# marwie/mageslam

Hardware: AMD Instinct MI355X
Metric: frames/sec ORB extract+match @720p; local-BA iters/sec (50 KF, 5k pts) (higher is better)
Workload: dtype u8

## Files before the change

### mageslam_amd/csrc/orb.hip

```cpp
#include <hip/hip_runtime.h>

#include <algorithm>
#include <cmath>
#include <cstring>
#include <type_traits>
#include <vector>

#include "common.hpp"
#include "cv_rng.hpp"
#include "fast_tile_plan.hpp"
#include "lds_sort.hpp"
#include "orb_tables.hpp"

namespace mage {
namespace {

constexpr int TW = 120, TH = 30;
constexpr int GX = (TW + 8) / 4;
constexpr int SR = 8;
constexpr int SROWS = TH + 2;
constexpr int LW = TW + 16;
constexpr int LH = TH + 8;
constexpr int FAST_THREADS = GX * (SROWS / SR);
constexpr int TCAP = (TW / 2) * (TH / 2);
// ... 11 lines not shown
    int dword_ok;
    int qword_ok;
    uint8_t* blur;
    int blur_stride;
    long long blur_pitch;
    int blur_bcols;
    const uint4* blur_ops;
    const int* gate;
    int* gate_next;
    uint32_t* redo;
};

struct Tile {
    int x, y;
};

__device__ __forceinline__ void wave_lds_sync()
{
    __builtin_amdgcn_fence(__ATOMIC_RELEASE, "wavefront");
    __builtin_amdgcn_wave_barrier();
    __builtin_amdgcn_fence(__ATOMIC_ACQUIRE, "wavefront");
}

typedef _Float16 h2 __attribute__((ext_vector_type(2)));
__device__ __forceinline__ h2 as_h2(uint32_t u) { return __builtin_bit_cast(h2, u); }
__device__ __forceinline__ uint32_t as_u32(h2 h) { return __builtin_bit_cast(uint32_t, h); }
__device__ __forceinline__ h2 min3h(h2 a, h2 b, h2 c)
{
    return __builtin_elementwise_minimum(__builtin_elementwise_minimum(a, b), c);
}
__device__ __forceinline__ h2 max3h(h2 a, h2 b, h2 c)
{
    return __builtin_elementwise_maximum(__builtin_elementwise_maximum(a, b), c);
}

__device__ __forceinline__ h2 pair_in(uint32_t d, int k)
{
    return as_h2(__builtin_amdgcn_perm(d, 0x64646464u, (uint32_t)((4 + k) | ((5 + k) << 16))));
}
__device__ __forceinline__ h2 pair_cross(uint32_t lo, uint32_t hi)
{
    return as_h2(__builtin_amdgcn_perm(hi, lo, 0x0C040C03u) | 0x64006400u);
}

__device__ __forceinline__ void window_row(uint32_t d0, uint32_t d1, uint32_t d2, h2 (&q)[9])
{
// ... 73 lines not shown
}

__device__ __forceinline__ int reflect101(int i, int n)
{
    if (n == 1) return 0;
    while ((unsigned)i >= (unsigned)n) i = i < 0 ? -i : 2 * n - 2 - i;
    return i;
}

typedef uint32_t u32x4 __attribute__((ext_vector_type(4)));
__device__ __forceinline__ u32x4 shr_bytes(u32x4 a, int s)
{
    if (s & 8) a = u32x4{a[2], a[3], 0u, 0u};
    if (s & 4) a = u32x4{a[1], a[2], a[3], 0u};
    const uint32_t b = (uint32_t)s & 3u;
    return u32x4{__builtin_amdgcn_alignbyte(a[1], a[0], b), __builtin_amdgcn_alignbyte(a[2], a[1], b),
                 __builtin_amdgcn_alignbyte(a[3], a[2], b), __builtin_amdgcn_alignbyte(0u, a[3], b)};
}
__device__ __forceinline__ u32x4 rev_bytes(u32x4 a)
{
    return u32x4{__builtin_bswap32(a[3]), __builtin_bswap32(a[2]), __builtin_bswap32(a[1]), __builtin_bswap32(a[0])};
}

__device__ __noinline__ void load_tile_border(const uint8_t* __restrict__ src_, int w_, int h_, int stride_,
                                              uint8_t (*img)[LW], int gx0_, int gy0_)
{
    const int w = __builtin_amdgcn_readfirstlane(w_), h = __builtin_amdgcn_readfirstlane(h_);
    const int stride = __builtin_amdgcn_readfirstlane(stride_);
    const int gx0 = __builtin_amdgcn_readfirstlane(gx0_), gy0 = __builtin_amdgcn_readfirstlane(gy0_);
    const unsigned long long sa = (unsigned long long)src_;
    const unsigned long long sb = ((unsigned long long)(uint32_t)__builtin_amdgcn_readfirstlane((int)(sa >> 32)) << 32) |
                                  (uint32_t)__builtin_amdgcn_readfirstlane((int)sa);
    typedef const __attribute__((address_space(1))) uint8_t* gptr;
    typedef uint32_t u32x2 __attribute__((ext_vector_type(2)));
    typedef const __attribute__((address_space(1))) u32x2 __attribute__((aligned(1))) g_u2;
    typedef const __attribute__((address_space(1))) u32x4 __attribute__((aligned(1))) g_u4;
    const gptr src = (gptr)sb;
    static_assert(LW == tileplan::kLW && LH == tileplan::kLH, "the plan's tile window");
    constexpr int RSTEP = FAST_THREADS / 9, NPASS = (LH + RSTEP - 1) / RSTEP;
    const int c = threadIdx.x % 9, r0 = threadIdx.x / 9;
    if (r0 >= RSTEP) return;
    if (gx0 + LW <= w) {
        const bool left = gx0 < 0 && c == 0;
        const gptr gc = src + (left ? 0 : gx0 + (c < 8 ? 16 * c : 120));
        u32x4 v[NPASS];
#pragma unroll
        for (int k = 0; k < NPASS; k++)
            if (r0 + k * RSTEP < LH)
                v[k] = *(g_u4*)(gc + (long long)tileplan::mirror1(gy0 + r0 + k * RSTEP, h) * stride);
#pragma unroll
        for (int k = 0; k < NPASS; k++) {
            const int r = r0 + k * RSTEP;
            if (r >= LH) break;
            u32x4 t = v[k];
            if (left)
                t = u32x4{__builtin_amdgcn_perm(t[2], t[1], 0x01020304u), __builtin_amdgcn_perm(t[1], t[0], 0x01020304u),
                          t[0], t[1]};
            uint2* d = reinterpret_cast<uint2*>(&img[r][16 * c]);
            if (c < 8) {
                d[0] = make_uint2(t[0], t[1]);
                d[1] = make_uint2(t[2], t[3]);
            } else {
                d[0] = make_uint2(t[2], t[3]);
// ... 21 lines not shown
#pragma unroll
        for (int k = 0; k < NPASS; k++) {
            const int r = r0 + k * RSTEP;
            if (r >= LH) break;
            const u32x4 t = v[k];
            u32x4 o;
            if (cp.kind == tileplan::CHUNK_STRADDLE) {
                o = shr_bytes(t, 16 - cp.n) | rev_bytes(shr_bytes(t, cp.n - 1));
            } else if (cp.kind == tileplan::CHUNK_MIRROR) {
                o = half ? u32x4{__builtin_bswap32(t[1]), __builtin_bswap32(t[0]), 0u, 0u} : rev_bytes(t);
            } else if (cp.kind == tileplan::CHUNK_LEFT) {
                o = u32x4{__builtin_amdgcn_perm(t[2], t[1], 0x01020304u), __builtin_amdgcn_perm(t[1], t[0], 0x01020304u),
                          t[0], t[1]};
            } else {
                o = c < 8 ? t : u32x4{t[2], t[3], 0u, 0u};
            }
            uint2* d = reinterpret_cast<uint2*>(&img[r][16 * c]);
            d[0] = make_uint2(o[0], o[1]);
            if (c < 8) d[1] = make_uint2(o[2], o[3]);
        }
    }
}

__device__ __forceinline__ void load_tile(const uint8_t* __restrict__ src, const FastParams& p,
                                          uint8_t (*img)[LW], Tile T)
{
    const int gx0 = T.x * TW - 8, gy0 = T.y * TH - 4;
    if (p.qword_ok && gx0 >= 0 && gx0 + LW <= p.w && gy0 >= 0 && gy0 + LH <= p.h) {
        static_assert(LW == 8 * 16 + 8, "row = 8 x 16 + 8 bytes");
        constexpr int RSTEP = FAST_THREADS / 9, NPASS = (LH + RSTEP - 1) / RSTEP;
        const int c = threadIdx.x % 9, r0 = threadIdx.x / 9;
        if (r0 < RSTEP) {
            const uint8_t* g = src + (long long)(gy0 + r0) * p.stride + gx0 + (c < 8 ? 16 * c : 120);
            const long long gstep = (long long)RSTEP * p.stride;
            typedef uint32_t u32x4 __attribute__((ext_vector_type(4)));
            u32x4 v[NPASS];
#pragma unroll
            for (int k = 0; k < NPASS; k++)
                if (r0 + k * RSTEP < LH) __builtin_memcpy(&v[k], g + k * gstep, 16);
#pragma unroll
            for (int k = 0; k < NPASS; k++) {
                const int r = r0 + k * RSTEP;
                if (r >= LH) break;
                if (c < 8) {
                    uint2* d = reinterpret_cast<uint2*>(&img[r][16 * c]);
                    d[0] = make_uint2(v[k][0], v[k][1]);
                    d[1] = make_uint2(v[k][2], v[k][3]);
                } else {
                    *reinterpret_cast<uint2*>(&img[r][128]) = make_uint2(v[k][2], v[k][3]);
                }
            }
        }
        return;
    }
    if (p.qword_ok && tileplan::border_ok(p.w, p.h, gx0, gy0)) {
        load_tile_border(src, p.w, p.h, p.stride, img, gx0, gy0);
        return;
    }
    constexpr int DW = LW / 4;
    for (int i = threadIdx.x; i < LH * DW; i += FAST_THREADS) {
        const int r = i / DW, c = i - r * DW;
        const int gx = gx0 + 4 * c, gy = reflect101(gy0 + r, p.h);
        const uint8_t* row = src + (long long)gy * p.stride;
        uint32_t v;
        if (p.dword_ok && gx >= 0 && gx + 3 < p.w) {
            v = *reinterpret_cast<const uint32_t*>(row + gx);
        } else {
            v = 0;
#pragma unroll
            for (int q = 0; q < 4; q++) v |= (uint32_t)row[reflect101(gx + q, p.w)] << (8 * q);
        }
        *reinterpret_cast<uint32_t*>(&img[r][4 * c]) = v;
    }
}

__device__ __forceinline__ void score_strip(const uint8_t (*img)[LW], uint32_t (*sc)[GX], const FastParams& p, Tile T)
{
    const int gx = threadIdx.x % GX, chunk = threadIdx.x / GX;
    const int X0 = T.x * TW - 4 + 4 * gx;
    const int Y0 = T.y * TH - 1 + SR * chunk;
    uint32_t colmask = 0;
#pragma unroll
    for (int q = 0; q < 4; q++)
        if (X0 + q >= 3 && X0 + q <= p.w - 4) colmask |= 0xFFu << (8 * q);
    const _Float16 t = (_Float16)(float)p.threshold;
    const h2 tf = {t, t};
    const uint32_t* base = reinterpret_cast<const uint32_t*>(&img[SR * chunk][0]) + gx;
    h2 win[7][9];
#pragma unroll
    for (int r = 0; r < 6; r++) {
        const uint32_t* rp = base + r * (LW / 4);
        window_row(rp[0], rp[1], rp[2], win[r + 1]);
    }
    uint32_t nx0 = base[6 * (LW / 4)], nx1 = base[6 * (LW / 4) + 1], nx2 = base[6 * (LW / 4) + 2];
#pragma unroll
    for (int r = 0; r < SR; r++) {
#pragma unroll
        for (int k = 0; k < 6; k++)
#pragma unroll
            for (int i = 0; i < 9; i++) win[k][i] = win[k + 1][i];
        window_row(nx0, nx1, nx2, win[6]);
// ... 185 lines not shown
            uint32_t t[4];
#pragma unroll
            for (int r = 0; r < 4; r++) t[r] = ((uint32_t)yh[r] << 8) + (uint32_t)yl[r];
            const u16x2 cap = {255, 255};
            const uint32_t h01 = __builtin_bit_cast(uint32_t, __builtin_elementwise_min(
                __builtin_bit_cast(u16x2, __builtin_amdgcn_perm(t[1], t[0], 0x07060302u)), cap));
            const uint32_t h23 = __builtin_bit_cast(uint32_t, __builtin_elementwise_min(
                __builtin_bit_cast(u16x2, __builtin_amdgcn_perm(t[3], t[2], 0x07060302u)), cap));
            const uint32_t w = __builtin_amdgcn_perm(h23, h01, 0x06040200u);
            if (yok[o] && xok) *reinterpret_cast<uint32_t*>(fb + (off + (o ? ostep : 0u))) = w;
        }
    }
}

#ifndef MAGE_FAST_WAVES_PER_EU
#define MAGE_FAST_WAVES_PER_EU 6
#endif
#ifndef MAGE_FAST_STAMPS
#define MAGE_FAST_STAMPS 0
#endif
#if MAGE_FAST_STAMPS
__device__ unsigned long long g_fast_stamps[4096][2][16];
#define FAST_STAMP(k)                                                                                   \
    if ((threadIdx.x & 63) == 0 && f < 15) {                                                           \
        const int t_ = f * p.tiles + T.y * p.tiles_x + T.x;              \
        if (t_ < 4096) g_fast_stamps[t_][threadIdx.x >> 6][k] = __builtin_amdgcn_s_memtime();           \
    }
#else
#define FAST_STAMP(k)
#endif
template <bool kMayGate>
__device__ __forceinline__ void fast_tile(const uint8_t* __restrict__ frames, const FastParams& p, int f, int G,
                                          bool blur, uint32_t* __restrict__ cand, uint32_t* __restrict__ counts,
                                          Tile T)
{
    __shared__ __attribute__((aligned(16))) uint8_t img[LH][LW];
    __shared__ uint32_t sc[SROWS][GX];
    const int tix = T.y * p.tiles_x + T.x;
    uint32_t* const tile_out = cand + (long long)f * p.cand_cap + (long long)tix * TCAP;
    uint32_t* const list = tile_out;
    constexpr uint32_t ICAP = 512;
    __shared__ __attribute__((aligned(4))) uint16_t items[FAST_THREADS / kWave][ICAP];
    __shared__ uint32_t s_cnt, s_dense;
    FAST_STAMP(0);
    load_tile(frames + (long long)f * p.pitch, p, img, T);
    if (threadIdx.x == 0) s_cnt = s_dense = 0;
    __syncthreads();
    FAST_STAMP(1);
    const bool gated = kMayGate && G > p.threshold;
    uint32_t total = 0;
    if (gated) {
        const uint32_t pix = gate_strip(img, sc, G, p, T);
        FAST_STAMP(2);
        const uint32_t cnt = __builtin_popcount(pix);
        uint32_t pre = 0;
#pragma unroll
        for (int j = 0; j < 6; j++) {
            const uint64_t b = __ballot((cnt >> j) & 1u);
            pre += __builtin_amdgcn_mbcnt_hi((uint32_t)(b >> 32), __builtin_amdgcn_mbcnt_lo((uint32_t)b, 0u)) << j;
            total += (uint32_t)__builtin_popcountll(b) << j;
        }
        if (total > ICAP) {
            if (__lane_id() == 0) s_dense = 1u;
        } else {
            uint16_t* wl = items[threadIdx.x / kWave];
            const uint32_t ibase = threadIdx.x << 5;
            uint32_t rb = pix;
            while (rb) {
                const int b = __builtin_ctz(rb);
// ... 15 lines not shown
            for (uint32_t i0 = 0; i0 < total; i0 += 2 * kWave) {
                const uint32_t i = i0 + 2 * __lane_id();
                uint32_t ia = 0, ib = 0;
                bool fa = false, fb = false;
                if (i < total) {
                    const uint32_t pr = *reinterpret_cast<const uint32_t*>(&wl[i]);
                    ia = pr & 0xFFFFu;
                    ib = i + 1 < total ? pr >> 16 : ia;
                    const uint32_t ss = score_pixels(img, scb, ia, ib, tg, tg1);
                    fa = (ss & 0xFFu) != 0;
                    fb = i + 1 < total && (ss >> 16) != 0;
                }
                const uint64_t ba = __ballot(fa), bb = __ballot(fb);
                const uint32_t below = __builtin_amdgcn_mbcnt_hi((uint32_t)(ba >> 32), __builtin_amdgcn_mbcnt_lo((uint32_t)ba, 0u)) +
                                       __builtin_amdgcn_mbcnt_hi((uint32_t)(bb >> 32), __builtin_amdgcn_mbcnt_lo((uint32_t)bb, 0u));
                const uint32_t pa = nz + below;
                if (fa) wl[pa] = (uint16_t)ia;
                if (fb) wl[pa + (fa ? 1u : 0u)] = (uint16_t)ib;
                nz += (uint32_t)(__builtin_popcountll(ba) + __builtin_popcountll(bb));
            }
            total = nz;
            FAST_STAMP(5);
        }
    } else {
        score_strip(img, sc, p, T);
    }
    FAST_STAMP(6);
    if (blur) blur_mfma(img, p, f, T);
    FAST_STAMP(7);
    __syncthreads();
    if (gated && !s_dense) {
        const uint16_t* wl = items[threadIdx.x / kWave];
        const uint8_t* scb = reinterpret_cast<const uint8_t*>(&sc[0][0]);
        constexpr int RB = 4 * GX;
        for (uint32_t i0 = 0; i0 < total; i0 += kWave) {
            const uint32_t i = i0 + __lane_id();
            bool m = false;
            uint32_t c = 0;
            if (i < total) {
                const uint32_t it = wl[i];
                const int sr = (int)item_row(it), x = (int)item_col(it);
                const int X = T.x * TW + x - 4, Y = T.y * TH + sr - 1;
                if (sr >= 1 && sr <= TH && x >= 4 && x < TW + 4 && X >= p.xlo && X <= p.xhi && Y >= p.ylo &&
                    Y <= p.yhi) {
                    const uint8_t* q = scb + sr * RB + x;
                    const uint32_t v = q[0];
                    const uint32_t nb = max(max(max(q[-RB - 1], q[-RB]), max(q[-RB + 1], q[-1])),
                                            max(max(q[1], q[RB - 1]), max(q[RB], q[RB + 1])));
                    m = v > nb;
                    c = ((uint32_t)Y << 20) | ((uint32_t)X << 8) | v;
                }
            }
            const uint64_t b = __ballot(m);
            if (b) {
                uint32_t base = 0;
                if (__lane_id() == 0) base = atomicAdd(&s_cnt, (uint32_t)__builtin_popcountll(b));
                base = __builtin_amdgcn_readfirstlane(base);
                const uint32_t pre = __builtin_amdgcn_mbcnt_hi((uint32_t)(b >> 32), __builtin_amdgcn_mbcnt_lo((uint32_t)b, 0u));
                if (m) list[base + pre] = c;
            }
        }
    } else {
        constexpr int OG = TW / 4;
        const int og = threadIdx.x % 32, chunk = threadIdx.x / 32;
        const int X0 = T.x * TW + 4 * og;
        const int oy0 = 8 * chunk, oy1 = min(oy0 + 8, TH);
        uint32_t bits = 0;
        if (og < OG) {
            uint32_t colbits = 0;
#pragma unroll
            for (int q = 0; q < 4; q++)
                if (X0 + q >= p.xlo && X0 + q <= p.xhi) colbits |= 1u << q;
            auto even = [](uint32_t d) { return as_h2(__builtin_amdgcn_perm(d, 0x64646464u, 0x00060004u)); };
            auto odd = [](uint32_t d) { return as_h2(__builtin_amdgcn_perm(d, 0x64646464u, 0x00070005u)); };
            struct RowV {
                h2 ce, co, le, lo, re, ro, he, ho;
            };
            auto load_row = [&](int srow) {
                RowV v;
                const uint32_t l = sc[srow][og], c = sc[srow][og + 1], r = sc[srow][og + 2];
                const uint32_t L = __builtin_amdgcn_alignbyte(c, l, 3), R = __builtin_amdgcn_alignbyte(r, c, 1);
                v.ce = even(c);
                v.co = odd(c);
                v.le = even(L);
                v.lo = odd(L);
                v.re = even(R);
                v.ro = odd(R);
                v.he = max3h(v.le, v.ce, v.re);
                v.ho = max3h(v.lo, v.co, v.ro);
                return v;
            };
// ... 17 lines not shown
        for (int j = 0; j < 6; j++) {
            const uint64_t b = __ballot((cnt >> j) & 1u);
            pre += __builtin_amdgcn_mbcnt_hi((uint32_t)(b >> 32), __builtin_amdgcn_mbcnt_lo((uint32_t)b, 0u)) << j;
            total += (uint32_t)__builtin_popcountll(b) << j;
        }
        if (total) {
            uint32_t base = 0;
            if (__lane_id() == 0) base = atomicAdd(&s_cnt, total);
            uint32_t idx = __builtin_amdgcn_readfirstlane(base) + pre;
            const uint8_t* scb = reinterpret_cast<const uint8_t*>(&sc[0][0]);
            while (bits) {
                const int b = __builtin_ctz(bits);
                bits &= bits - 1u;
                const int oy = oy0 + (b >> 2), q = b & 3;
                const uint32_t sv = scb[(oy + 1) * (4 * GX) + 4 * (og + 1) + q];
                list[idx++] = ((uint32_t)(T.y * TH + oy) << 20) | ((uint32_t)(X0 + q) << 8) | sv;
            }
        }
    }
    FAST_STAMP(8);
    __syncthreads();
    FAST_STAMP(11);
    const uint32_t n = s_cnt;
    if (threadIdx.x == 0) counts[(long long)f * p.tiles + tix] = n;
    FAST_STAMP(12);
}

__global__ __launch_bounds__(FAST_THREADS, MAGE_FAST_WAVES_PER_EU) void fast_nms_kernel(const uint8_t* __restrict__ frames,
                                                                FastParams p,
                                                                uint32_t* __restrict__ cand,
                                                                uint32_t* __restrict__ counts)
{
    const int G = p.gate ? *p.gate : 0;
    if (p.gate_next && (blockIdx.x | blockIdx.y | blockIdx.z | threadIdx.x) == 0) {
        *p.gate_next = 255;
        p.redo[0] = 0;
    }
    fast_tile<true>(frames, p, blockIdx.z, G, p.blur != nullptr, cand, counts, Tile{(int)blockIdx.x, (int)blockIdx.y});
}

constexpr int REDO_BLOCKS = 64;
__global__ __launch_bounds__(FAST_THREADS, 4) void fast_redo_kernel(const uint8_t* __restrict__ frames,
                                                                 FastParams p,
                                                                 uint32_t* __restrict__ cand,
                                                                 uint32_t* __restrict__ counts)
{
    const uint32_t n = p.redo[0], tiles = (uint32_t)p.tiles;
    for (uint32_t w = blockIdx.x; w < n * tiles; w += gridDim.x) {
        const uint32_t z = w / tiles, t = w - z * tiles;
        const int ty = (int)(t / (uint32_t)p.tiles_x), tx = (int)t - ty * p.tiles_x;
        fast_tile<false>(frames, p, (int)p.redo[1 + z], 0, false, cand, counts, Tile{tx, ty});
        __syncthreads();
    }
}

__global__ __launch_bounds__(FAST_THREADS) void fast_score_map_kernel(const uint8_t* __restrict__ src,
                                                                      FastParams p,
                                                                      uint8_t* __restrict__ score)
{
    __shared__ __attribute__((aligned(16))) uint8_t img[LH][LW];
    __shared__ uint32_t sc[SROWS][GX];
    const Tile T{(int)blockIdx.x, (int)blockIdx.y};
    load_tile(src, p, img, T);
    __syncthreads();
    score_strip(img, sc, p, T);
    __syncthreads();
    const uint8_t* scb = reinterpret_cast<const uint8_t*>(&sc[0][0]);
    for (int i = threadIdx.x; i < TW * TH; i += FAST_THREADS) {
        const int oy = i / TW, ox = i - oy * TW;
        const int X = blockIdx.x * TW + ox, Y = blockIdx.y * TH + oy;
        if (X >= p.w || Y >= p.h) continue;
        score[(long long)Y * p.w + X] = scb[(oy + 1) * (4 * GX) + ox + 4];
    }
}
// ... 26 lines not shown

enum : uint32_t { ST_KMAX = 1u, ST_CELLS = 2u };

__device__ __forceinline__ int cand_x(uint32_t c) { return (int)((c >> 8) & 0xFFFu); }
__device__ __forceinline__ int cand_y(uint32_t c) { return (int)(c >> 20); }
__device__ __forceinline__ int cand_s(uint32_t c) { return (int)(c & 0xFFu); }

static_assert(SEL_THREADS == SORT_THREADS, "select_kernel sorts with the shared LDS sort");

#ifndef MAGE_SELECT_STAMPS
#define MAGE_SELECT_STAMPS 0
#endif
#if MAGE_SELECT_STAMPS
__device__ unsigned long long g_sel_stamps[1024][16];
#define SEL_STAMP(k) \
    if (threadIdx.x == 0 && f < 1024) g_sel_stamps[f][k] = __builtin_amdgcn_s_memtime()
#else
#define SEL_STAMP(k)
#endif

#ifndef MAGE_GATE_SHIFT
#define MAGE_GATE_SHIFT 4
#endif
__device__ __forceinline__ void select_frame(int f, int G, const uint32_t* __restrict__ cand,
                                             const uint32_t* __restrict__ counts, const SelectParams& p,
                                             mage_keypoint* __restrict__ kp_out, uint32_t* __restrict__ xy_out,
                                             uint32_t* __restrict__ n_out, uint32_t* __restrict__ status)
{
    __shared__ uint32_t hist[256];
    __shared__ uint32_t items[KMAX];
    __shared__ uint32_t sorted[KMAX];
    __shared__ uint32_t cellStart[CELLMAX + 1];
    __shared__ unsigned long long keys[KMAX];
    __shared__ int s_cut, s_K, s_minX, s_maxX, s_minY, s_maxY, s_minS, s_gmax, s_mcd2, s_mode;
    __shared__ float s_rob, s_robInv;

    const int tid = threadIdx.x;
    SEL_STAMP(0);
    const uint32_t* C = cand + (long long)f * p.cand_cap;
    const uint32_t* CNT = counts + (long long)f * p.tiles;
    const int base = p.accumulate ? (int)n_out[f] : 0;
    for (int i = tid; i < 256; i += SEL_THREADS) hist[i] = 0;
    if (tid == 0) {
        s_K = 0;
        s_minX = s_minY = s_minS = 0x7FFFFFFF;
        s_maxX = s_maxY = -1;
    }
    const int T = p.tiles;
    uint32_t* tstart = sorted;
    for (int t = tid; t < T; t += SEL_THREADS) tstart[t] = min(CNT[t], (uint32_t)TCAP);
    __syncthreads();
    if (tid < kWave) {
        const int per = (T + kWave) / kWave;
        const int b0 = tid * per, b1 = min(b0 + per, T + 1);
        uint32_t sum = 0;
        for (int i = b0; i < b1; i++) sum += i < T ? tstart[i] : 0u;
// ... 59 lines not shown
#pragma unroll
        for (int j = 0; j < 4; j++) {
            if (sfx[j] + above >= N) hiN = 4 * tid + j;
            if (sfx[j] + above >= p.max_num) hiM = 4 * tid + j;
        }
#pragma unroll
        for (int m = 32; m >= 1; m >>= 1) {
            hiN = max(hiN, __shfl_xor(hiN, m));
            hiM = max(hiM, __shfl_xor(hiM, m));
        }
        if (tid == 0) {
            int lower = 0;
            if (n0 <= N) {
                s_mode = 0;
                s_cut = 0;
            } else {
                const int minNumThreshold = hiN >= minThreshold ? hiN : minThreshold;
                lower = max((int)__fmul_rn((float)minNumThreshold, p.feature_strength), minThreshold);
                s_cut = max(hiM, lower);
                s_mode = 1;
            }
            if (G > p.fast_threshold && (s_mode == 0 || lower < G)) {
                s_mode = 2;
                const uint32_t k = atomicAdd(&p.redo[0], 1u);
                p.redo[1 + k] = (uint32_t)f;
            } else if (p.gate_next) {
                atomicMin(p.gate_next, s_mode == 1 ? lower - (lower >> MAGE_GATE_SHIFT) : 0);
            }
        }
    }
    __syncthreads();
    SEL_STAMP(3);
    if (s_mode == 2) return;
    const int cut = s_cut;
    for_each_cand([&](uint32_t c) {
        if (cand_s(c) >= cut) {
            const int pos = atomicAdd(&s_K, 1);
            if (pos < KMAX) items[pos] = c;
        }
    });
    __syncthreads();
    SEL_STAMP(4);
    int K = s_K;
    if (K > KMAX) {
        if (tid == 0) atomicOr(status, ST_KMAX);
        K = KMAX;
    }
    int P = 1;
    while (P < K) P <<= 1;
    const bool anms = s_mode == 1 && N <= K;

    if (!anms) {
        for (int i = tid; i < P; i += SEL_THREADS) {
            unsigned long long key = 0;
            if (i < K) {
                uint32_t c = items[i];
                uint32_t raster = (uint32_t)cand_y(c) * (uint32_t)p.w + (uint32_t)cand_x(c);
                key = ((unsigned long long)(0xFFFFFFFFu - raster) << 8) | (unsigned long long)cand_s(c);
            }
            keys[i] = key;
        }
        __syncthreads();
        sort_desc(keys, P);
    } else {
        const int numX = p.cells_x, numY = p.cells_y, ncell = numX * numY;
        if (ncell > CELLMAX) {
            if (tid == 0) {
                atomicOr(status, ST_CELLS);
                n_out[f] = (uint32_t)base;
            }
            return;
        }
        {
            int mnX = 0x7FFFFFFF, mxX = -1, mnY = 0x7FFFFFFF, mxY = -1, mnS = 0x7FFFFFFF;
            for (int i = tid; i < K; i += SEL_THREADS) {
                const uint32_t c = items[i];
                mnX = min(mnX, cand_x(c));
                mxX = max(mxX, cand_x(c));
                mnY = min(mnY, cand_y(c));
                mxY = max(mxY, cand_y(c));
                mnS = min(mnS, cand_s(c));
            }
#pragma unroll
            for (int m = 32; m >= 1; m >>= 1) {
                mnX = min(mnX, __shfl_xor(mnX, m));
                mxX = max(mxX, __shfl_xor(mxX, m));
                mnY = min(mnY, __shfl_xor(mnY, m));
                mxY = max(mxY, __shfl_xor(mxY, m));
                mnS = min(mnS, __shfl_xor(mnS, m));
            }
            if ((tid & (kWave - 1)) == 0 && mxX >= 0) {
                atomicMin(&s_minX, mnX);
                atomicMax(&s_maxX, mxX);
                atomicMin(&s_minY, mnY);
// ... 213 lines not shown
        uint32_t raster, s;
        if (anms) {
            raster = 0xFFFFFFFFu - (uint32_t)(key & 0xFFFFFFFFull);
            s = (uint32_t)((key >> 32) & 0xFFu);
        } else {
            raster = 0xFFFFFFFFu - (uint32_t)(key >> 8);
            s = (uint32_t)(key & 0xFFu);
        }
        uint32_t y = raster / (uint32_t)p.w, x = raster - y * (uint32_t)p.w;
        mage_keypoint k;
        k.x = __fmul_rn((float)x, p.scale);
        k.y = __fmul_rn((float)y, p.scale);
        k.size = p.kp_size;
        k.angle = 0.0f;
        k.response = (float)s;
        k.octave = p.level;
        k.class_id = -1;
        kp[i] = k;
        xy[i] = (y << 16) | x;
        if (lv) lv[i] = (uint16_t)(p.level << 8);
    }
    if (tid == 0) n_out[f] = (uint32_t)(base + nout);
    SEL_STAMP(10);
}

__global__ __launch_bounds__(SEL_THREADS) void select_kernel(const uint32_t* __restrict__ cand,
                                                             const uint32_t* __restrict__ counts, SelectParams p,
                                                             mage_keypoint* __restrict__ kp_out,
                                                             uint32_t* __restrict__ xy_out,
                                                             uint32_t* __restrict__ n_out,
                                                             uint32_t* __restrict__ status)
{
    select_frame(blockIdx.x, p.gate ? *p.gate : 0, cand, counts, p, kp_out, xy_out, n_out, status);
}

__global__ __launch_bounds__(SEL_THREADS) void select_redo_kernel(const uint32_t* __restrict__ cand,
                                                                  const uint32_t* __restrict__ counts, SelectParams p,
                                                                  mage_keypoint* __restrict__ kp_out,
                                                                  uint32_t* __restrict__ xy_out,
                                                                  uint32_t* __restrict__ n_out,
                                                                  uint32_t* __restrict__ status)
{
    const uint32_t n = p.redo[0];
    for (uint32_t z = blockIdx.x; z < n; z += gridDim.x) {
        select_frame((int)p.redo[1 + z], 0, cand, counts, p, kp_out, xy_out, n_out, status);
        __syncthreads();
    }
}

constexpr int DESC_WAVES = 4;
constexpr int RMAX = 18;
constexpr int KHMAX = 7;

struct LevelImages {
    const uint8_t* base[MAGE_MAX_LEVELS];
    long long pitch[MAGE_MAX_LEVELS];
    int stride[MAGE_MAX_LEVELS];
};

struct DescParams {
    LevelImages lev;
    int lw[MAGE_MAX_LEVELS], lh[MAGE_MAX_LEVELS];
    const uint16_t* lvl;
    unsigned out_cap;
    int R;
    int ksize;
    int taps[2 * KHMAX + 1];
    int dword_ok;
    int chunks, frames;
    int random;
// ... 739 lines not shown
    int area2 = 0;
    size_t xofs = 0, yofs = 0, alpha = 0, beta = 0;
};

struct Geometry {
    int w = -1, h = -1, L = 0;
    LevelGeom lv[MAGE_MAX_LEVELS];
    size_t pyr_bytes = 0, blur_bytes = 0, cand_total = 0, tile_total = 0;
    std::vector<int> tab_ints;
    std::vector<uint32_t> tab_words;
    bool tab_valid = false;
};

struct OrbDetector {
    mage_orb_settings s{};
    int device = 0;
    int taps[2 * KHMAX + 1] = {0};
    int R = 7;
    bool random_pattern = false;
    Geometry geo;
    DeviceBuffer pattern, cand, counts, xy, status, img, kp, desc, n, blurred, pyr, rtab, lvl, blur_ops;
    DeviceBuffer gates, redo;
    int gate_par = 0;
    uint32_t last_batch = 0;
};

void resize_tables(int sw, int sh, int dw, int dh, std::vector<int>& ints, std::vector<uint32_t>& words, LevelGeom& v)
{
    struct Dim { int w, h; };
    const Dim src{sw, sh}, dst{dw, dh};
    const double scale_x = 1. / ((double)dst.w / src.w), scale_y = 1. / ((double)dst.h / src.h);
    v.xmax = dst.w;
    v.xofs = ints.size();
    v.alpha = words.size();
    for (int dx = 0; dx < dst.w; dx++) {
        float fx = (float)((dx + 0.5) * scale_x - 0.5);
        int sx = (int)std::floor(fx);
        fx -= sx;
        if (sx < 0) fx = 0, sx = 0;
        if (sx + 1 >= src.w) {
            v.xmax = std::min(v.xmax, dx);
            if (sx >= src.w - 1) fx = 0, sx = src.w - 1;
        }
        ints.push_back(sx);
        const int a0 = (int)std::lrint((1.f - fx) * 2048), a1 = (int)std::lrint(fx * 2048);
        words.push_back((uint32_t)(uint16_t)a0 | ((uint32_t)(uint16_t)a1 << 16));
    }
// ... 185 lines not shown
    g.tab_valid = false;
}

mage_status run_batch(OrbDetector* o, const uint8_t* d_frames, uint32_t batch, int w, int h,
                      int stride, long long pitch, mage_keypoint* d_kp, uint8_t* d_desc,
                      uint32_t cap, uint32_t* d_n, hipStream_t st)
{
    const mage_orb_settings& s = o->s;
    Geometry& g = o->geo;
    if (g.w != w || g.h != h || g.L != (int)s.nlevels) level_geometry(o, w, h);
    const int L = g.L;
    MAGE_REQUIRE(g.lv[0].tiles < KMAX, MAGE_EUNSUPPORTED, "frame too large for the candidate tile table");
    const bool multi = L > 1 || s.use_orientation;
    mage_status r;
    if ((r = o->cand.reserve((size_t)batch * g.cand_total * 4)) != MAGE_OK) return r;
    if ((r = o->counts.reserve((size_t)batch * g.tile_total * 4)) != MAGE_OK) return r;
    if ((r = o->xy.reserve((size_t)batch * std::max(cap, 1u) * 4)) != MAGE_OK) return r;
    const bool fresh_status = o->status.ptr == nullptr;
    if ((r = o->status.reserve(4)) != MAGE_OK) return r;
    if (fresh_status) MAGE_HIP(hipMemsetAsync(o->status.ptr, 0, 4, st));
    const bool fresh_gates = o->gates.ptr == nullptr;
    if ((r = o->gates.reserve(2 * MAGE_MAX_LEVELS * sizeof(int))) != MAGE_OK) return r;
    if (fresh_gates) MAGE_HIP(hipMemsetAsync(o->gates.ptr, 0, 2 * MAGE_MAX_LEVELS * sizeof(int), st));
    if ((r = o->redo.reserve((size_t)L * (1 + batch) * 4)) != MAGE_OK) return r;
    o->last_batch = batch;
    int* gate_cur = o->gates.as<int>() + o->gate_par * MAGE_MAX_LEVELS;
    int* gate_nxt = o->gates.as<int>() + (1 - o->gate_par) * MAGE_MAX_LEVELS;
    o->gate_par ^= 1;
    if (multi && (r = o->lvl.reserve((size_t)batch * std::max(cap, 1u) * 2)) != MAGE_OK) return r;
    if (L > 1 && (r = o->pyr.reserve((size_t)batch * g.pyr_bytes)) != MAGE_OK) return r;
    if (!g.tab_valid && L > 1) {
        const size_t ib = g.tab_ints.size() * 4, wb = g.tab_words.size() * 4;
        if ((r = o->rtab.reserve(ib + wb)) != MAGE_OK) return r;
        MAGE_HIP(hipMemcpy(o->rtab.ptr, g.tab_ints.data(), ib, hipMemcpyHostToDevice));
        MAGE_HIP(hipMemcpy(o->rtab.as<uint8_t>() + ib, g.tab_words.data(), wb, hipMemcpyHostToDevice));
        g.tab_valid = true;
    }

    LevelImages raw{};
    for (int l = 0; l < L; l++) {
        if (l == 0) {
            raw.base[0] = d_frames;
            raw.pitch[0] = pitch;
            raw.stride[0] = stride;
        } else {
            raw.base[l] = o->pyr.as<uint8_t>() + (size_t)batch * g.lv[l].off;
            raw.pitch[l] = g.lv[l].pitch;
            raw.stride[l] = g.lv[l].stride;
// ... 52 lines not shown
        fp.threshold = std::min(std::max((int)s.fast_threshold, 0), 255);
        fp.xlo = std::max(3, border);
        fp.xhi = std::min(W - 4, W - border - 1);
        fp.ylo = std::max(3, border);
        fp.yhi = std::min(H - 4, H - border - 1);
        if (H <= 2 * border || W <= 2 * border) fp.xhi = -1;
        fp.cand_cap = v.cand_cap;
        fp.tiles = v.tiles;
        fp.tiles_x = (W + TW - 1) / TW;
        fp.dword_ok = (fp.stride % 4 == 0) && (fp.pitch % 4 == 0) && ((uintptr_t)raw.base[l] % 4 == 0);
        fp.qword_ok = (fp.stride % 8 == 0) && (fp.pitch % 8 == 0) && ((uintptr_t)raw.base[l] % 8 == 0);
        if (fused_blur) {
            blurred.base[l] = o->blurred.as<uint8_t>() + (size_t)batch * v.boff;
            blurred.pitch[l] = v.bpitch;
            blurred.stride[l] = v.bcols;
            fp.blur = const_cast<uint8_t*>(blurred.base[l]);
            fp.blur_stride = v.stride;
            fp.blur_pitch = v.bpitch;
            fp.blur_bcols = v.bcols;
            fp.blur_ops = o->blur_ops.as<uint4>();
        }
        uint32_t* cand = o->cand.as<uint32_t>() + (size_t)batch * v.coff;
        uint32_t* counts = o->counts.as<uint32_t>() + (size_t)batch * v.toff;
        uint32_t* redo = o->redo.as<uint32_t>() + (size_t)l * (1 + batch);
        fp.gate = gate_cur + l;
        fp.gate_next = gate_nxt + l;
        fp.redo = redo;
        const dim3 fgrid((W + TW - 1) / TW, (H + TH - 1) / TH, batch);
        launch("orb.fast_nms", fast_nms_kernel, fgrid, dim3(FAST_THREADS), 0, st, raw.base[l], fp, cand, counts);
        MAGE_HIP(hipGetLastError());

        SelectParams sp{};
        sp.w = W;
        sp.h = H;
        sp.cand_cap = v.cand_cap;
        sp.tiles = v.tiles;
        sp.nfeatures = v.nfeatures;
        sp.max_num = (int)((float)v.nfeatures * s.feature_factor);
        sp.out_cap = cap;
        sp.fast_threshold = (int)s.fast_threshold;
        sp.feature_strength = s.feature_strength;
        sp.strong = s.strong_response;
        sp.min_r = s.min_robust_factor;
        sp.max_r = s.max_robust_factor;
        sp.cells_x = s.num_cells_x;
        sp.cells_y = s.num_cells_y;
        sp.kp_size = (float)s.patch_size * v.scale;
        sp.level = l;
        sp.scale = v.scale;
        sp.accumulate = l > 0;
        sp.lvl = multi ? o->lvl.as<uint16_t>() : nullptr;
        sp.gate = gate_cur + l;
        sp.gate_next = gate_nxt + l;
        sp.redo = redo;
        launch("orb.select", select_kernel, dim3(batch), dim3(SEL_THREADS), 0, st, cand, counts, sp, d_kp,
               o->xy.as<uint32_t>(), d_n, o->status.as<uint32_t>());
        MAGE_HIP(hipGetLastError());
        launch("orb.fast_redo", fast_redo_kernel, dim3(REDO_BLOCKS), dim3(FAST_THREADS), 0,
               st, raw.base[l], fp, cand, counts);
        launch("orb.select_redo", select_redo_kernel, dim3(std::min(batch, 8u)), dim3(SEL_THREADS), 0, st, cand,
               counts, sp, d_kp, o->xy.as<uint32_t>(), d_n, o->status.as<uint32_t>());
        MAGE_HIP(hipGetLastError());
    }

    if (cap > 0 && s.use_orientation) {
        OrientParams op{};
        op.lev = raw;
        op.out_cap = cap;
        op.half_k = half;
        int vmax = (int)std::floor(half * std::sqrt(2.f) / 2 + 1), vmin = (int)std::ceil(half * std::sqrt(2.f) / 2);
        for (int v = 0; v <= vmax; ++v) op.umax[v] = (int)std::lrint(std::sqrt((double)half * half - v * v));
        for (int v = half, v0 = 0; v >= vmin; --v) {
            while (op.umax[v0] == op.umax[v0 + 1]) ++v0;
            op.umax[v] = v0;
            ++v0;
        }
        if (half >= 5 && half <= 15)
        {
            op.chunks = (int)((cap + ORIENT_PER_BLOCK - 1) / ORIENT_PER_BLOCK);
            op.frames = (int)batch;
            launch("orb.orient", orient_rows_kernel, dim3((unsigned)(op.chunks * ((batch + 7) / 8) * 8)), dim3(256), 0, st,
                   d_kp, o->xy.as<uint32_t>(), o->lvl.as<uint16_t>(), d_n, op);
        }
        else
// ... 326 lines not shown
    if (fresh) MAGE_HIP(hipMemsetAsync(orb->gates.ptr, 0, 2 * MAGE_MAX_LEVELS * sizeof(int), st));
    int* slot = orb->gates.as<int>() + orb->gate_par * MAGE_MAX_LEVELS + level;
    MAGE_HIP(hipMemcpyAsync(slot, &gate, sizeof(int), hipMemcpyHostToDevice, st));
    MAGE_HIP(hipStreamSynchronize(st));
    return MAGE_OK;
}

mage_status mage_orb_fast_gate_stats(mage_orb* orb, uint32_t level, int32_t* last_gate, int32_t* next_gate,
                                     uint32_t* last_redo, mage_stream stream)
{
    MAGE_REQUIRE(orb && level < MAGE_MAX_LEVELS && last_gate && next_gate && last_redo, MAGE_EINVAL, "bad arguments");
    MAGE_HIP(hipSetDevice(orb->device));
    *last_gate = *next_gate = 0;
    *last_redo = 0;
    if (!orb->gates.ptr) return MAGE_OK;
    hipStream_t st = (hipStream_t)stream;
    const int* g = orb->gates.as<int>();
    MAGE_HIP(hipMemcpyAsync(last_gate, g + (1 - orb->gate_par) * MAGE_MAX_LEVELS + level, sizeof(int),
                            hipMemcpyDeviceToHost, st));
    MAGE_HIP(hipMemcpyAsync(next_gate, g + orb->gate_par * MAGE_MAX_LEVELS + level, sizeof(int),
                            hipMemcpyDeviceToHost, st));
    const int L = orb->geo.L;
    if (orb->redo.ptr && (int)level < L)
        MAGE_HIP(hipMemcpyAsync(last_redo, orb->redo.as<uint32_t>() + (size_t)level * (1 + orb->last_batch), 4,
                                hipMemcpyDeviceToHost, st));
    MAGE_HIP(hipStreamSynchronize(st));
    return MAGE_OK;
}

mage_status mage_debug_fast_tile_plan(const uint8_t* img, int32_t w, int32_t h, int32_t stride, int32_t tx,
                                      int32_t ty, int32_t* path, int32_t* loads, uint8_t* tile)
{
    namespace tp = mage::tileplan;
    MAGE_REQUIRE(path && loads && w > 0 && h > 0 && stride >= w && tx >= 0 && ty >= 0 && tx * mage::TW < w &&
                     ty * mage::TH < h && (!img || tile), MAGE_EINVAL, "bad arguments");
    const int gx0 = tx * mage::TW - 8, gy0 = ty * mage::TH - 4;
    const bool qword_ok = stride % 8 == 0;
    const bool interior = gx0 >= 0 && gx0 + mage::LW <= w && gy0 >= 0 && gy0 + mage::LH <= h;
    *path = !qword_ok ? 0 : interior ? 1 : tp::border_ok(w, h, gx0, gy0) ? 2 : 0;
    if (*path == 0) return MAGE_OK;
    for (int r = 0; r < mage::LH; r++)
        for (int c = 0; c < tp::kChunks; c++) {
            const tp::ChunkPlan cp = tp::chunk_plan(w, gx0, c);
            const long long off = (long long)tp::mirror1(gy0 + r, h) * stride + cp.x;
            const int nb = tp::load_bytes(cp);
            loads[(r * tp::kChunks + c) * 2] = (int32_t)off;
            loads[(r * tp::kChunks + c) * 2 + 1] = nb;
// ... 90 lines not shown
```

Baseline: 431,900.

## Fold FAST redo and reselect into select kernel using per-team LDS aliasing

Removes the separate fast_redo and select_redo launches per pyramid level. When a frame's selection decides it needs a redo, the same select block runs the FAST tiles for that frame itself, split across eight 128-thread teams whose LDS aliases the select kernel's item/sort/key pool, and then reselects. The goal is to cut two kernel launches per level and the global redo frame list. The cost is that redo work for a frame is now serialized inside one block instead of spread over 64 blocks. The select kernel also gets larger, which may raise register or LDS pressure.

```diff
diff --git a/mageslam_amd/csrc/orb.hip b/mageslam_amd/csrc/orb.hip
--- a/mageslam_amd/csrc/orb.hip
+++ b/mageslam_amd/csrc/orb.hip
@@ -57,6 +57,12 @@
     __builtin_amdgcn_fence(__ATOMIC_ACQUIRE, "wavefront");
 }
 
+template <bool kTeam>
+__device__ __forceinline__ unsigned fast_tid()
+{
+    return kTeam ? threadIdx.x & (unsigned)(FAST_THREADS - 1) : threadIdx.x;
+}
+
 typedef _Float16 h2 __attribute__((ext_vector_type(2)));
 __device__ __forceinline__ h2 as_h2(uint32_t u) { return __builtin_bit_cast(h2, u); }
 __device__ __forceinline__ uint32_t as_u32(h2 h) { return __builtin_bit_cast(uint32_t, h); }
@@ -176,6 +182,7 @@
     return u32x4{__builtin_bswap32(a[3]), __builtin_bswap32(a[2]), __builtin_bswap32(a[1]), __builtin_bswap32(a[0])};
 }
 
+template <bool kTeam>
 __device__ __noinline__ void load_tile_border(const uint8_t* __restrict__ src_, int w_, int h_, int stride_,
                                               uint8_t (*img)[LW], int gx0_, int gy0_)
 {
@@ -192,7 +199,7 @@
     const gptr src = (gptr)sb;
     static_assert(LW == tileplan::kLW && LH == tileplan::kLH, "the plan's tile window");
     constexpr int RSTEP = FAST_THREADS / 9, NPASS = (LH + RSTEP - 1) / RSTEP;
-    const int c = threadIdx.x % 9, r0 = threadIdx.x / 9;
+    const int c = fast_tid<kTeam>() % 9, r0 = fast_tid<kTeam>() / 9;
     if (r0 >= RSTEP) return;
     if (gx0 + LW <= w) {
         const bool left = gx0 < 0 && c == 0;
@@ -260,6 +267,7 @@
     }
 }
 
+template <bool kTeam = false>
 __device__ __forceinline__ void load_tile(const uint8_t* __restrict__ src, const FastParams& p,
                                           uint8_t (*img)[LW], Tile T)
 {
@@ -267,7 +275,7 @@
     if (p.qword_ok && gx0 >= 0 && gx0 + LW <= p.w && gy0 >= 0 && gy0 + LH <= p.h) {
         static_assert(LW == 8 * 16 + 8, "row = 8 x 16 + 8 bytes");
         constexpr int RSTEP = FAST_THREADS / 9, NPASS = (LH + RSTEP - 1) / RSTEP;
-        const int c = threadIdx.x % 9, r0 = threadIdx.x / 9;
+        const int c = fast_tid<kTeam>() % 9, r0 = fast_tid<kTeam>() / 9;
         if (r0 < RSTEP) {
             const uint8_t* g = src + (long long)(gy0 + r0) * p.stride + gx0 + (c < 8 ? 16 * c : 120);
             const long long gstep = (long long)RSTEP * p.stride;
@@ -292,11 +300,11 @@
         return;
     }
     if (p.qword_ok && tileplan::border_ok(p.w, p.h, gx0, gy0)) {
-        load_tile_border(src, p.w, p.h, p.stride, img, gx0, gy0);
+        load_tile_border<kTeam>(src, p.w, p.h, p.stride, img, gx0, gy0);
         return;
     }
     constexpr int DW = LW / 4;
-    for (int i = threadIdx.x; i < LH * DW; i += FAST_THREADS) {
+    for (int i = fast_tid<kTeam>(); i < LH * DW; i += FAST_THREADS) {
         const int r = i / DW, c = i - r * DW;
         const int gx = gx0 + 4 * c, gy = reflect101(gy0 + r, p.h);
         const uint8_t* row = src + (long long)gy * p.stride;
@@ -312,9 +320,10 @@
     }
 }
 
+template <bool kTeam = false>
 __device__ __forceinline__ void score_strip(const uint8_t (*img)[LW], uint32_t (*sc)[GX], const FastParams& p, Tile T)
 {
-    const int gx = threadIdx.x % GX, chunk = threadIdx.x / GX;
+    const int gx = fast_tid<kTeam>() % GX, chunk = fast_tid<kTeam>() / GX;
     const int X0 = T.x * TW - 4 + 4 * gx;
     const int Y0 = T.y * TH - 1 + SR * chunk;
     uint32_t colmask = 0;
@@ -546,29 +555,43 @@
 #if MAGE_FAST_STAMPS
 __device__ unsigned long long g_fast_stamps[4096][2][16];
 #define FAST_STAMP(k)                                                                                   \
-    if ((threadIdx.x & 63) == 0 && f < 15) {                                                           \
+    if (!kTeam && (threadIdx.x & 63) == 0 && f < 15) {                                                 \
         const int t_ = f * p.tiles + T.y * p.tiles_x + T.x;              \
         if (t_ < 4096) g_fast_stamps[t_][threadIdx.x >> 6][k] = __builtin_amdgcn_s_memtime();           \
     }
 #else
 #define FAST_STAMP(k)
 #endif
-template <bool kMayGate>
+struct TeamLds {
+    uint8_t (*img)[LH][LW];
+    uint32_t (*sc)[SROWS][GX];
+    uint32_t* cnt;
+};
+template <bool kMayGate, bool kTeam = false>
 __device__ __forceinline__ void fast_tile(const uint8_t* __restrict__ frames, const FastParams& p, int f, int G,
                                           bool blur, uint32_t* __restrict__ cand, uint32_t* __restrict__ counts,
-                                          Tile T)
-{
-    __shared__ __attribute__((aligned(16))) uint8_t img[LH][LW];
-    __shared__ uint32_t sc[SROWS][GX];
+                                          Tile T, const TeamLds* team = nullptr, bool live = true)
+{
+    static_assert(!(kMayGate && kTeam), "the gated path's barriers are conditional");
+    constexpr uint32_t ICAP = 512;
+    __shared__ __attribute__((aligned(16))) uint8_t s_img[LH][LW];
+    __shared__ uint32_t s_sc[SROWS][GX];
+    __shared__ __attribute__((aligned(4))) uint16_t items[FAST_THREADS / kWave][ICAP];
+    __shared__ uint32_t s_cnt_, s_dense;
+    uint8_t (&img)[LH][LW] = kTeam ? *team->img : s_img;
+    uint32_t (&sc)[SROWS][GX] = kTeam ? *team->sc : s_sc;
+    uint32_t& s_cnt = kTeam ? *team->cnt : s_cnt_;
     const int tix = T.y * p.tiles_x + T.x;
     uint32_t* const tile_out = cand + (long long)f * p.cand_cap + (long long)tix * TCAP;
     uint32_t* const list = tile_out;
-    constexpr uint32_t ICAP = 512;
-    __shared__ __attribute__((aligned(4))) uint16_t items[FAST_THREADS / kWave][ICAP];
-    __shared__ uint32_t s_cnt, s_dense;
     FAST_STAMP(0);
-    load_tile(frames + (long long)f * p.pitch, p, img, T);
-    if (threadIdx.x == 0) s_cnt = s_dense = 0;
+    if (!kTeam || live) load_tile<kTeam>(frames + (long long)f * p.pitch, p, img, T);
+    if (fast_tid<kTeam>() == 0) {
+        if constexpr (kTeam)
+            s_cnt = 0;
+        else
+            s_cnt = s_dense = 0;
+    }
     __syncthreads();
     FAST_STAMP(1);
     const bool gated = kMayGate && G > p.threshold;
@@ -630,11 +653,11 @@
             total = nz;
             FAST_STAMP(5);
         }
-    } else {
-        score_strip(img, sc, p, T);
+    } else if (!kTeam || live) {
+        score_strip<kTeam>(img, sc, p, T);
     }
     FAST_STAMP(6);
-    if (blur) blur_mfma(img, p, f, T);
+    if (!kTeam && blur) blur_mfma(img, p, f, T);
     FAST_STAMP(7);
     __syncthreads();
     if (gated && !s_dense) {
@@ -670,11 +693,11 @@
         }
     } else {
         constexpr int OG = TW / 4;
-        const int og = threadIdx.x % 32, chunk = threadIdx.x / 32;
+        const int og = fast_tid<kTeam>() % 32, chunk = fast_tid<kTeam>() / 32;
         const int X0 = T.x * TW + 4 * og;
         const int oy0 = 8 * chunk, oy1 = min(oy0 + 8, TH);
         uint32_t bits = 0;
-        if (og < OG) {
+        if (og < OG && (!kTeam || live)) {
             uint32_t colbits = 0;
 #pragma unroll
             for (int q = 0; q < 4; q++)
@@ -738,7 +761,7 @@
     __syncthreads();
     FAST_STAMP(11);
     const uint32_t n = s_cnt;
-    if (threadIdx.x == 0) counts[(long long)f * p.tiles + tix] = n;
+    if ((!kTeam || live) && fast_tid<kTeam>() == 0) counts[(long long)f * p.tiles + tix] = n;
     FAST_STAMP(12);
 }
 
@@ -750,22 +773,29 @@
     const int G = p.gate ? *p.gate : 0;
     if (p.gate_next && (blockIdx.x | blockIdx.y | blockIdx.z | threadIdx.x) == 0) {
         *p.gate_next = 255;
-        p.redo[0] = 0;
+        *p.redo = 0;
     }
     fast_tile<true>(frames, p, blockIdx.z, G, p.blur != nullptr, cand, counts, Tile{(int)blockIdx.x, (int)blockIdx.y});
 }
 
-constexpr int REDO_BLOCKS = 64;
-__global__ __launch_bounds__(FAST_THREADS, 4) void fast_redo_kernel(const uint8_t* __restrict__ frames,
-                                                                 FastParams p,
-                                                                 uint32_t* __restrict__ cand,
-                                                                 uint32_t* __restrict__ counts)
-{
-    const uint32_t n = p.redo[0], tiles = (uint32_t)p.tiles;
-    for (uint32_t w = blockIdx.x; w < n * tiles; w += gridDim.x) {
-        const uint32_t z = w / tiles, t = w - z * tiles;
-        const int ty = (int)(t / (uint32_t)p.tiles_x), tx = (int)t - ty * p.tiles_x;
-        fast_tile<false>(frames, p, (int)p.redo[1 + z], 0, false, cand, counts, Tile{tx, ty});
+constexpr int REDO_TEAMS = 8;
+constexpr int REDO_IMG_BYTES = LH * LW, REDO_SC_BYTES = SROWS * GX * 4;
+constexpr int REDO_TEAM_LDS = (REDO_IMG_BYTES + REDO_SC_BYTES + 4 + 15) & ~15;
+static_assert(REDO_IMG_BYTES % 16 == 0, "the score rows stay 16-byte aligned behind the image window");
+__device__ __forceinline__ void redo_frame_tiles(const uint8_t* __restrict__ frames, const FastParams& p, int f,
+                                                 uint32_t* cand, uint32_t* counts, uint8_t* pool)
+{
+    const int team = (int)(threadIdx.x / FAST_THREADS);
+    uint8_t* const blk = pool + team * REDO_TEAM_LDS;
+    TeamLds lds;
+    lds.img = reinterpret_cast<uint8_t (*)[LH][LW]>(blk);
+    lds.sc = reinterpret_cast<uint32_t (*)[SROWS][GX]>(blk + REDO_IMG_BYTES);
+    lds.cnt = reinterpret_cast<uint32_t*>(blk + REDO_IMG_BYTES + REDO_SC_BYTES);
+    for (int t0 = 0; t0 < p.tiles; t0 += REDO_TEAMS) {
+        const bool live = t0 + team < p.tiles;
+        const int t = live ? t0 + team : 0;
+        const int ty = t / p.tiles_x, tx = t - ty * p.tiles_x;
+        fast_tile<false, true>(frames, p, f, 0, false, cand, counts, Tile{tx, ty}, &lds, live);
         __syncthreads();
     }
 }
@@ -838,16 +868,19 @@
 #ifndef MAGE_GATE_SHIFT
 #define MAGE_GATE_SHIFT 4
 #endif
-__device__ __forceinline__ void select_frame(int f, int G, const uint32_t* __restrict__ cand,
-                                             const uint32_t* __restrict__ counts, const SelectParams& p,
+constexpr int SEL_POOL_BYTES = KMAX * (4 + 4 + 8);
+static_assert(REDO_TEAMS * FAST_THREADS == SEL_THREADS, "eight 128-thread teams");
+static_assert(REDO_TEAMS * REDO_TEAM_LDS <= SEL_POOL_BYTES, "the team blocks alias items / sorted / keys");
+__device__ __forceinline__ bool select_frame(int f, int G, const uint32_t* cand, const uint32_t* counts,
+                                             const SelectParams& p, uint8_t* pool,
                                              mage_keypoint* __restrict__ kp_out, uint32_t* __restrict__ xy_out,
                                              uint32_t* __restrict__ n_out, uint32_t* __restrict__ status)
 {
     __shared__ uint32_t hist[256];
-    __shared__ uint32_t items[KMAX];
-    __shared__ uint32_t sorted[KMAX];
     __shared__ uint32_t cellStart[CELLMAX + 1];
-    __shared__ unsigned long long keys[KMAX];
+    uint32_t* const items = reinterpret_cast<uint32_t*>(pool);
+    uint32_t* const sorted = items + KMAX;
+    unsigned long long* const keys = reinterpret_cast<unsigned long long*>(pool + 2 * KMAX * 4);
     __shared__ int s_cut, s_K, s_minX, s_maxX, s_minY, s_maxY, s_minS, s_gmax, s_mcd2, s_mode;
     __shared__ float s_rob, s_robInv;
 
@@ -953,8 +986,7 @@
             }
             if (G > p.fast_threshold && (s_mode == 0 || lower < G)) {
                 s_mode = 2;
-                const uint32_t k = atomicAdd(&p.redo[0], 1u);
-                p.redo[1 + k] = (uint32_t)f;
+                atomicAdd(p.redo, 1u);
             } else if (p.gate_next) {
                 atomicMin(p.gate_next, s_mode == 1 ? lower - (lower >> MAGE_GATE_SHIFT) : 0);
             }
@@ -962,7 +994,7 @@
     }
     __syncthreads();
     SEL_STAMP(3);
-    if (s_mode == 2) return;
+    if (s_mode == 2) return true;
     const int cut = s_cut;
     for_each_cand([&](uint32_t c) {
         if (cand_s(c) >= cut) {
@@ -1000,7 +1032,7 @@
                 atomicOr(status, ST_CELLS);
                 n_out[f] = (uint32_t)base;
             }
-            return;
+            return false;
         }
         {
             int mnX = 0x7FFFFFFF, mxX = -1, mnY = 0x7FFFFFFF, mxY = -1, mnS = 0x7FFFFFFF;
@@ -1260,30 +1292,40 @@
     }
     if (tid == 0) n_out[f] = (uint32_t)(base + nout);
     SEL_STAMP(10);
-}
-
-__global__ __launch_bounds__(SEL_THREADS) void select_kernel(const uint32_t* __restrict__ cand,
-                                                             const uint32_t* __restrict__ counts, SelectParams p,
-                                                             mage_keypoint* __restrict__ kp_out,
-                                                             uint32_t* __restrict__ xy_out,
-                                                             uint32_t* __restrict__ n_out,
-                                                             uint32_t* __restrict__ status)
-{
-    select_frame(blockIdx.x, p.gate ? *p.gate : 0, cand, counts, p, kp_out, xy_out, n_out, status);
-}
-
-__global__ __launch_bounds__(SEL_THREADS) void select_redo_kernel(const uint32_t* __restrict__ cand,
-                                                                  const uint32_t* __restrict__ counts, SelectParams p,
-                                                                  mage_keypoint* __restrict__ kp_out,
-                                                                  uint32_t* __restrict__ xy_out,
-                                                                  uint32_t* __restrict__ n_out,
-                                                                  uint32_t* __restrict__ status)
-{
-    const uint32_t n = p.redo[0];
-    for (uint32_t z = blockIdx.x; z < n; z += gridDim.x) {
-        select_frame((int)p.redo[1 + z], 0, cand, counts, p, kp_out, xy_out, n_out, status);
-        __syncthreads();
-    }
+    return false;
+}
+
+struct SelectArgs {
+    const uint8_t* frames;
+    FastParams fp;
+    uint32_t* cand;
+    uint32_t* counts;
+    SelectParams p;
+    mage_keypoint* kp_out;
+    uint32_t* xy_out;
+    uint32_t* n_out;
+    uint32_t* status;
+};
+
+template <class T>
+__device__ __forceinline__ const T* kernel_arguments()
+{
+#if defined(__HIP_DEVICE_COMPILE__)
+    return reinterpret_cast<const T*>(__builtin_amdgcn_kernarg_segment_ptr());
+#else
+    return nullptr;
+#endif
+}
+
+__global__ __launch_bounds__(SEL_THREADS) void select_kernel(SelectArgs a)
+{
+    __shared__ __attribute__((aligned(16))) uint8_t pool[SEL_POOL_BYTES];
+    const int f = blockIdx.x;
+    if (!select_frame(f, a.p.gate ? *a.p.gate : 0, a.cand, a.counts, a.p, pool, a.kp_out, a.xy_out, a.n_out, a.status))
+        return;
+    const SelectArgs* ka = kernel_arguments<SelectArgs>();
+    redo_frame_tiles(ka->frames, ka->fp, f, ka->cand, ka->counts, pool);
+    select_frame(f, 0, ka->cand, ka->counts, ka->p, pool, ka->kp_out, ka->xy_out, ka->n_out, ka->status);
 }
 
 constexpr int DESC_WAVES = 4;
@@ -2069,7 +2111,6 @@
     DeviceBuffer pattern, cand, counts, xy, status, img, kp, desc, n, blurred, pyr, rtab, lvl, blur_ops;
     DeviceBuffer gates, redo;
     int gate_par = 0;
-    uint32_t last_batch = 0;
 };
 
 void resize_tables(int sw, int sh, int dw, int dh, std::vector<int>& ints, std::vector<uint32_t>& words, LevelGeom& v)
@@ -2301,8 +2342,7 @@
     const bool fresh_gates = o->gates.ptr == nullptr;
     if ((r = o->gates.reserve(2 * MAGE_MAX_LEVELS * sizeof(int))) != MAGE_OK) return r;
     if (fresh_gates) MAGE_HIP(hipMemsetAsync(o->gates.ptr, 0, 2 * MAGE_MAX_LEVELS * sizeof(int), st));
-    if ((r = o->redo.reserve((size_t)L * (1 + batch) * 4)) != MAGE_OK) return r;
-    o->last_batch = batch;
+    if ((r = o->redo.reserve((size_t)L * 4)) != MAGE_OK) return r;
     int* gate_cur = o->gates.as<int>() + o->gate_par * MAGE_MAX_LEVELS;
     int* gate_nxt = o->gates.as<int>() + (1 - o->gate_par) * MAGE_MAX_LEVELS;
     o->gate_par ^= 1;
@@ -2401,7 +2441,7 @@
         }
         uint32_t* cand = o->cand.as<uint32_t>() + (size_t)batch * v.coff;
         uint32_t* counts = o->counts.as<uint32_t>() + (size_t)batch * v.toff;
-        uint32_t* redo = o->redo.as<uint32_t>() + (size_t)l * (1 + batch);
+        uint32_t* redo = o->redo.as<uint32_t>() + l;
         fp.gate = gate_cur + l;
         fp.gate_next = gate_nxt + l;
         fp.redo = redo;
@@ -2432,13 +2472,8 @@
         sp.gate = gate_cur + l;
         sp.gate_next = gate_nxt + l;
         sp.redo = redo;
-        launch("orb.select", select_kernel, dim3(batch), dim3(SEL_THREADS), 0, st, cand, counts, sp, d_kp,
-               o->xy.as<uint32_t>(), d_n, o->status.as<uint32_t>());
-        MAGE_HIP(hipGetLastError());
-        launch("orb.fast_redo", fast_redo_kernel, dim3(REDO_BLOCKS), dim3(FAST_THREADS), 0,
-               st, raw.base[l], fp, cand, counts);
-        launch("orb.select_redo", select_redo_kernel, dim3(std::min(batch, 8u)), dim3(SEL_THREADS), 0, st, cand,
-               counts, sp, d_kp, o->xy.as<uint32_t>(), d_n, o->status.as<uint32_t>());
+        launch("orb.select", select_kernel, dim3(batch), dim3(SEL_THREADS), 0, st,
+               SelectArgs{raw.base[l], fp, cand, counts, sp, d_kp, o->xy.as<uint32_t>(), d_n, o->status.as<uint32_t>()});
         MAGE_HIP(hipGetLastError());
     }
 
@@ -2811,7 +2846,7 @@
                             hipMemcpyDeviceToHost, st));
     const int L = orb->geo.L;
     if (orb->redo.ptr && (int)level < L)
-        MAGE_HIP(hipMemcpyAsync(last_redo, orb->redo.as<uint32_t>() + (size_t)level * (1 + orb->last_batch), 4,
+        MAGE_HIP(hipMemcpyAsync(last_redo, orb->redo.as<uint32_t>() + level, 4,
                                 hipMemcpyDeviceToHost, st));
     MAGE_HIP(hipStreamSynchronize(st));
     return MAGE_OK;
```

Result: no change. 434,500 (median of 6 runs) (+0.6%).
